# wdas03/lipreading-video-generation

Hardware: AMD Instinct MI355X
Metric: train-step frames/sec + DDIM steps/sec, 128x128x16 UNet3D at 1/2/4/8 GPUs (higher is better)
Workload: dtype bf16

## Files before the change

### include/vdiff.h

```cpp
#ifndef VDIFF_H
#define VDIFF_H

#include <stdint.h>
#include <stddef.h>

#ifdef __cplusplus
extern "C" {
#endif

#define VDIFF_ABI_VERSION 1

enum vd_status { VD_OK = 0, VD_EINVAL = 1, VD_EUNSUPPORTED = 2, VD_ELAUNCH = 3 };
enum vd_dtype { VD_F32 = 0, VD_BF16 = 1 };

int vd_version(void);
const char* vd_last_error(void);
int vd_device_info(char* buf, int buflen);

int vd_timestep_embedding(const int64_t* t, int B, int dim, float max_period,
                          float* out, void* stream);
int vd_timestep_embedding_tab(const int64_t* t, int B, int dim, const float* freqs,
                              float* out, void* stream);

int vd_q_sample(const void* x0, const void* eps, void* xt, const int64_t* t,
// ... 82 lines not shown
typedef struct vd_conv_desc {
  int B;
  int Ti, Hi, Wi, Ci;
  int To, Ho, Wo, Co;
  int kt, kh, kw;
  int st, sh, sw;
  int pt, ph, pw;
  int x_cstride;
  int y_cstride;
  int dtype;
} vd_conv_desc;

int vd_conv3d_fwd(const vd_conv_desc* d, const void* x, const void* w_fwd,
                  const float* bias, const float* chan_add,
                  const void* residual, void* y, void* stream);
int vd_conv3d_bwd_data(const vd_conv_desc* d, const void* dy,
                       const void* w_bwd, void* dx, void* stream);
int vd_conv3d_bwd_weight(const vd_conv_desc* d, const void* x, const void* dy,
                         float* dw, void* stream);
size_t vd_conv3d_bwd_weight_workspace_size(const vd_conv_desc* d);
int vd_conv3d_bwd_weight_det(const vd_conv_desc* d, const void* x, const void* dy, float* dw,
                             int Co_out, int Ci_out, void* workspace, size_t workspace_bytes,
                             void* stream);

int vd_conv_set_wgrad(int mode);
int vd_conv_set_halo(int mode);

size_t vd_channel_sums_workspace_size(int B, int C);
int vd_channel_sums(const void* x, int B, int64_t S, int C, int cstride, int dtype,
                    float* out, void* workspace, void* stream);
int vd_conv_pack_weight(const float* w, int Co, int Ci, int taps, int Cip, int Cop,
                        int transpose, int dtype, void* out, void* stream);
typedef struct {
  const float* w;
  void* out;
  int Co, Ci, taps, Cip, Cop, transpose;
  int64_t start;
} vd_pack_desc;
int vd_conv_pack_weights(const vd_pack_desc* descs, int n, int64_t total, int dtype,
                         void* stream);

typedef struct vd_attn_desc {
  int nseq, seq_len, head_dim, groups;
  int64_t batch_stride, group_stride, token_stride;
  int64_t o_batch_stride, o_group_stride, o_token_stride;
  float scale;
// ... 71 lines not shown
```

### lipreading-video-generation_amd/csrc/conv.hip

```cpp
#include "vd_common.h"
#include <stdio.h>
#include <stdlib.h>

#include <atomic>

namespace {

constexpr int kThreads = 256;
constexpr int kBK = 32;

template <typename T> struct Cfg;
template <> struct Cfg<bf16_t> {
  static constexpr int EPC = 8;
  static constexpr int CPR = kBK / EPC;
  static constexpr int LDK = kBK;
};
template <> struct Cfg<float> {
  static constexpr int EPC = 4;
  static constexpr int CPR = kBK / EPC;
  static constexpr int LDK = kBK + 4;
};

__device__ __forceinline__ int swz(int r, int kc) {
  const int t = (r >> 2) & 3;
// ... 194 lines not shown
#pragma unroll
        for (int e = 0; e < 8; ++e) o[e] += rv[e];
      }
      store8(out, o);
    } else {
      for (int e = 0; e < lim; ++e) {
        float val = o[e];
        if (residual) val += Elem<T>::ld(residual + m * g.dNs + n + e);
        Elem<T>::st(out + e, val);
      }
    }
  }
}

struct WgtGeom {
  int B;
  int Ti, Hi, Wi, Ci, xCs;
  int To, Ho, Wo, Co, yCs;
  int kt, kh, kw, st, sh, sw, pt, ph, pw;
  int64_t M;
  int64_t m_per_split;
  int64_t split_stride;
  int xcd_tiles, xcd_total;
};

__device__ __forceinline__ bool wg_tile(const WgtGeom& g, int* tile, int* split) {
  if (g.xcd_tiles == 0) {
    *tile = blockIdx.x;
    *split = blockIdx.y;
    return true;
  }
  const int per = gridDim.x / 8;
  const int L = (blockIdx.x % 8) * per + blockIdx.x / 8;
  if (L >= g.xcd_total) return false;
  *tile = L % g.xcd_tiles;
  *split = L / g.xcd_tiles;
  return true;
}

__device__ __forceinline__ void wg_out(const WgtGeom& g, float* dw, int split, int64_t off,
                                       float v) {
  if (g.split_stride)
    dw[(int64_t)split * g.split_stride + off] = v;
  else
    atomicAdd(dw + off, v);
}

template <typename T>
__global__ __launch_bounds__(kThreads) void conv_wgrad_kernel(WgtGeom g, const T* __restrict__ x,
                                                              const T* __restrict__ dy,
                                                              float* __restrict__ dw) {
  constexpr int TM = 64, TN = 64;
  constexpr int PK = 32;
  constexpr int PAD = sizeof(T) == 2 ? 8 : 4;
  constexpr int LD = TM + PAD;
  constexpr int EPC = 16 / sizeof(T);
  constexpr int CPRW = TM / EPC;
  constexpr int CH = PK * CPRW / kThreads;
  constexpr int STAGE = 2 * PK * LD;
  extern __shared__ __attribute__((aligned(16))) char smem[];
  T* lds = reinterpret_cast<T*>(smem);

  const int taps = g.kt * g.kh * g.kw;
  const int co_tiles = (g.Co + TM - 1) / TM;
  const int ci_tiles = (g.Ci + TN - 1) / TN;
  int bid = blockIdx.x;
  const int cot = bid % co_tiles; bid /= co_tiles;
  const int cit = bid % ci_tiles; bid /= ci_tiles;
  const int tap = bid;
// ... 490 lines not shown
    const int tap = tab * g.kw + tc;
#pragma unroll
    for (int i = 0; i < 2; ++i)
#pragma unroll
      for (int j = 0; j < 2; ++j) {
        const int ci = ci0 + wn * 32 + 16 * j + fr;
        if (ci >= g.Ci) continue;
#pragma unroll
        for (int r = 0; r < 4; ++r) {
          const int co = co0 + wm * 32 + 16 * i + fq * 4 + r;
          if (co < g.Co) wg_out(g, dw, blockIdx.y, (int64_t)co * krow + (int64_t)tap * g.Ci + ci, acc[tc][i][j][r]);
        }
      }
  }
}

__device__ __forceinline__ int wg_swz(int r) {
  const int u = r >> 1;
  return ((u + 2 * (u >> 2)) & 3) << 1;
}
__device__ __forceinline__ int wg_off(int r, int c) {
  return r * 64 + ((((c >> 3) ^ wg_swz(r)) << 3) | (c & 7));
}

template <int RW, int COT, int NST, bool ONE, bool PLANE = false>
__global__ __launch_bounds__(kThreads, PLANE ? 1 : 2) void wgrad_dma_kernel(
    WgtGeom g, int wc, const bf16_t* __restrict__ x, const bf16_t* __restrict__ dy,
    float* __restrict__ dw) {
  constexpr int PY = COT / 32, PX = RW / 32;
  constexpr int PIECES = PY + PX;
  constexpr int Y_BYTES = COT * 128, STAGE = (COT + RW) * 128;
  constexpr int WTM = COT / 2, NI = WTM / 16;
  constexpr int NT = ONE ? 1 : (PLANE ? 9 : 3);
  static_assert(!PLANE || RW >= 3 * 66, "plane: three strip rows of 66 pixels");
  static_assert(!ONE || RW == 64, "1x1: the X tile is the step's 64 pixels");
  extern __shared__ __attribute__((aligned(16))) char smem[];
  const bf16_t* lds = reinterpret_cast<const bf16_t*>(smem);

  const int co_tiles = (g.Co + COT - 1) / COT, ci_tiles = (g.Ci + 63) / 64;
  int bid, wsplit;
  if (!wg_tile(g, &bid, &wsplit)) return;
  const int cot = bid % co_tiles; bid /= co_tiles;
  const int cit = bid % ci_tiles; bid /= ci_tiles;
  const int tab = bid;
  const int ta = PLANE ? tab : tab / g.kh, tb = PLANE ? 0 : tab % g.kh;
  const int co0 = cot * COT, ci0 = cit * 64;
// ... 87 lines not shown
      cw += 64;
      while (cw >= g.Wo) {
        cw -= g.Wo;
        if (++chh == g.Ho) {
          chh = 0;
          if (++ct == g.To) {
            ct = 0;
            ++cb;
          }
        }
      }
    }
  };

  const int wm = wave & 1, wn = wave >> 1;
  f32x4 acc[NT][NI][2];
#pragma unroll
  for (int tc = 0; tc < NT; ++tc)
#pragma unroll
    for (int i = 0; i < NI; ++i)
#pragma unroll
      for (int j = 0; j < 2; ++j) acc[tc][i][j] = f32x4{0.f, 0.f, 0.f, 0.f};

  vm_drain();
#pragma unroll
  for (int s = 0; s < NST - 1; ++s) issue(s);
  const int fr = lane & 15, fq = lane >> 4, q4 = fr >> 2, p4 = fr & 3;
  for (int s = 0; s < nsteps; ++s) {
    vm_wait_barrier<(NST - 2) * PIECES>();
    issue(s + NST - 1);
    const bf16_t* Ys = lds + (s % NST) * (STAGE / 2);
    const bf16_t* Xs = Ys + Y_BYTES / 2;
#pragma unroll
    for (int ks = 0; ks < 2; ++ks) {
      const int p_lo = 32 * ks + 8 * fq + q4, p_hi = p_lo + 4;
      bf16x8 af[NI];
#pragma unroll
      for (int i = 0; i < NI; ++i) {
        const int c = wm * WTM + 16 * i + 4 * p4;
        const bf16_t* plane = Ys + (c >> 6) * 4096;
        const bf16x4 lo = __builtin_amdgcn_ds_read_tr16_b64_v4i16(
            (lds_bf16x4*)(plane + wg_off(p_lo, c & 63)));
        const bf16x4 hi = __builtin_amdgcn_ds_read_tr16_b64_v4i16(
            (lds_bf16x4*)(plane + wg_off(p_hi, c & 63)));
        af[i] = bf16x8{lo[0], lo[1], lo[2], lo[3], hi[0], hi[1], hi[2], hi[3]};
      }
      const int s_lo = ONE ? p_lo : (p_lo / wc) * SW + p_lo % wc;
      const int s_hi = ONE ? p_hi : (p_hi / wc) * SW + p_hi % wc;
#pragma unroll
      for (int tc = 0; tc < NT; ++tc) {
        bf16x8 bfr[2];
        const int sh_t = PLANE ? (tc / 3) * SW + tc % 3 : tc;
#pragma unroll
        for (int j = 0; j < 2; ++j) {
          const int c = wn * 32 + 16 * j + 4 * p4;
          const bf16x4 lo = __builtin_amdgcn_ds_read_tr16_b64_v4i16(
              (lds_bf16x4*)(Xs + wg_off(s_lo + sh_t, c)));
          const bf16x4 hi = __builtin_amdgcn_ds_read_tr16_b64_v4i16(
              (lds_bf16x4*)(Xs + wg_off(s_hi + sh_t, c)));
          bfr[j] = bf16x8{lo[0], lo[1], lo[2], lo[3], hi[0], hi[1], hi[2], hi[3]};
        }
#pragma unroll
        for (int i = 0; i < NI; ++i)
#pragma unroll
          for (int j = 0; j < 2; ++j)
            acc[tc][i][j] =
                __builtin_amdgcn_mfma_f32_16x16x32_bf16(af[i], bfr[j], acc[tc][i][j], 0, 0, 0);
      }
    }
  }
  vm_drain();
  const int taps = g.kt * g.kh * g.kw;
  const int64_t krow = (int64_t)taps * g.Ci;
#pragma unroll
  for (int tc = 0; tc < NT; ++tc) {
    const int tap = ONE ? 0 : (PLANE ? ta * 9 + tc : tab * g.kw + tc);
#pragma unroll
    for (int i = 0; i < NI; ++i)
#pragma unroll
      for (int j = 0; j < 2; ++j) {
        const int ci = ci0 + wn * 32 + 16 * j + fr;
        if (ci >= g.Ci) continue;
#pragma unroll
        for (int r = 0; r < 4; ++r) {
          const int co = co0 + wm * WTM + 16 * i + fq * 4 + r;
          if (co < g.Co) wg_out(g, dw, wsplit, (int64_t)co * krow + (int64_t)tap * g.Ci + ci, acc[tc][i][j][r]);
        }
      }
  }
}

template <int RW, int COT, int NST, int KIND, bool ER = true>
__global__ __launch_bounds__(kThreads, 2) void wgrad_strip_kernel(WgtGeom g, int wc,
                                                                  const bf16_t* __restrict__ x,
                                                                  const bf16_t* __restrict__ dy,
                                                                  float* __restrict__ dw) {
  constexpr int PY = COT / 32, PX = RW / 32;
  constexpr int PIECES = PY + PX;
  constexpr int Y_BYTES = COT * 128, STAGE = (COT + RW) * 128;
  constexpr bool ROW1 = KIND == 1, ONE = KIND == 2;
  constexpr int WTM = COT / 2, NI = WTM / 16, NT = ONE ? 1 : 3;
  static_assert(!ONE || RW == 64, "1x1: the X tile is the step's 64 pixels");
  extern __shared__ __attribute__((aligned(16))) char smem[];

  const int co_tiles = (g.Co + COT - 1) / COT, ci_tiles = (g.Ci + 63) / 64;
  int bid, wsplit;
  if (!wg_tile(g, &bid, &wsplit)) return;
  const int cot = bid % co_tiles; bid /= co_tiles;
  const int cit = bid % ci_tiles; bid /= ci_tiles;
  const int tab = bid;
  const int ta = tab / g.kh, tb = tab % g.kh;
  const int co0 = cot * COT, ci0 = cit * 64;
  const int64_t mbeg = (int64_t)wsplit * g.m_per_split;
  int64_t mend = mbeg + g.m_per_split;
  if (mend > g.M) mend = g.M;
  if (mbeg >= mend) return;

  const int tid = threadIdx.x, lane = tid & 63;
  const int wave = __builtin_amdgcn_readfirstlane(tid >> 6);
// ... 111 lines not shown
#pragma unroll
      for (int j = 0; j < 2; ++j) acc[tc][i][j] = f32x4{0.f, 0.f, 0.f, 0.f};
  const int fr = lane & 15, fq = lane >> 4, q4 = fr >> 2, p4 = fr & 3;
  const uint32_t lb = lds_addr(smem);
  uint32_t abase[2][2][NI], xbase[2][2][NT][2];
#pragma unroll
  for (int ks = 0; ks < 2; ++ks)
#pragma unroll
    for (int hl = 0; hl < 2; ++hl) {
      const int p = 32 * ks + 8 * fq + q4 + 4 * hl;
      const int sp = ONE ? p : (p / wc) * SW + p % wc;
#pragma unroll
      for (int i = 0; i < NI; ++i) {
        const int c = wm * WTM + 16 * i + 4 * p4;
        abase[ks][hl][i] = lb + ((c >> 6) * 4096 + wg_off(p, c & 63)) * 2;
      }
#pragma unroll
      for (int tc = 0; tc < NT; ++tc)
#pragma unroll
        for (int j = 0; j < 2; ++j)
          xbase[ks][hl][tc][j] = lb + Y_BYTES + wg_off(sp + tc, wn * 32 + 16 * j + 4 * p4) * 2;
    }

  vm_drain();
#pragma unroll
  for (int s = 0; s < NST - 1; ++s) issue(s, s);
  for (int s0 = 0; s0 < nsteps; s0 += NST) {
#pragma unroll
    for (int ks = 0; ks < 2; ++ks)
#pragma unroll
      for (int hl = 0; hl < 2; ++hl) {
#pragma unroll
        for (int i = 0; i < NI; ++i) asm volatile("" : "+v"(abase[ks][hl][i]));
#pragma unroll
        for (int tc = 0; tc < NT; ++tc)
#pragma unroll
          for (int j = 0; j < 2; ++j) asm volatile("" : "+v"(xbase[ks][hl][tc][j]));
      }
#pragma unroll
    for (int u = 0; u < NST; ++u) {
      const int s = s0 + u;
      if (s >= nsteps) break;
      vm_lgk_wait_barrier<(NST - 2) * PIECES>();
      issue(s + NST - 1, (u + NST - 1) % NST);
#pragma unroll
      for (int ks = 0; ks < 2; ++ks) {
        bf16x8 af[NI], bfr[NT][2];
        auto rd = [&](uint32_t a0, uint32_t a1) {
          const bf16x4 lo = __builtin_amdgcn_ds_read_tr16_b64_v4i16(
              (lds_bf16x4*)(uintptr_t)(a0 + u * STAGE));
          const bf16x4 hi = __builtin_amdgcn_ds_read_tr16_b64_v4i16(
              (lds_bf16x4*)(uintptr_t)(a1 + u * STAGE));
          return bf16x8{lo[0], lo[1], lo[2], lo[3], hi[0], hi[1], hi[2], hi[3]};
        };
#pragma unroll
        for (int i = 0; i < NI; ++i) af[i] = rd(abase[ks][0][i], abase[ks][1][i]);
        if constexpr (ER) {
#pragma unroll
          for (int tc = 0; tc < NT; ++tc)
#pragma unroll
            for (int j = 0; j < 2; ++j) bfr[tc][j] = rd(xbase[ks][0][tc][j], xbase[ks][1][tc][j]);
          __builtin_amdgcn_sched_barrier(0);
        }
#pragma unroll
        for (int tc = 0; tc < NT; ++tc) {
          if constexpr (!ER) {
#pragma unroll
            for (int j = 0; j < 2; ++j) bfr[tc][j] = rd(xbase[ks][0][tc][j], xbase[ks][1][tc][j]);
          }
#pragma unroll
          for (int i = 0; i < NI; ++i)
#pragma unroll
            for (int j = 0; j < 2; ++j)
              acc[tc][i][j] = __builtin_amdgcn_mfma_f32_16x16x32_bf16(af[i], bfr[tc][j],
                                                                      acc[tc][i][j], 0, 0, 0);
        }
      }
    }
  }
  vm_drain();
  const int taps = g.kt * g.kh * g.kw;
  const int64_t krow = (int64_t)taps * g.Ci;
#pragma unroll
  for (int tc = 0; tc < NT; ++tc) {
    const int tap = ONE ? 0 : tab * g.kw + tc;
#pragma unroll
    for (int i = 0; i < NI; ++i)
#pragma unroll
      for (int j = 0; j < 2; ++j) {
        const int ci = ci0 + wn * 32 + 16 * j + fr;
        if (ci >= g.Ci) continue;
#pragma unroll
        for (int r = 0; r < 4; ++r) {
          const int co = co0 + wm * WTM + 16 * i + fq * 4 + r;
          if (co < g.Co)
            wg_out(g, dw, wsplit, (int64_t)co * krow + (int64_t)tap * g.Ci + ci,
                   acc[tc][i][j][r]);
        }
      }
  }
}

template <int BM, int BN, int WAVES_M, bool TR, int NST>
__global__ __launch_bounds__(kThreads, 2) void igemm_dma_kernel(
    GemmGeom g, const bf16_t* __restrict__ src, const bf16_t* __restrict__ wt,
    bf16_t* __restrict__ dst, const float* __restrict__ bias, const float* __restrict__ chan_add,
    const bf16_t* __restrict__ residual) {
  constexpr int WAVES_N = 4 / WAVES_M;
  constexpr int WTM = BM / WAVES_M, WTN = BN / WAVES_N;
  constexpr int NI = WTM / 16, NJ = WTN / 16;
  constexpr int IA = BM / 32, IB = BN / 32;
  constexpr int PIECES = IA + IB;
  constexpr int A_BYTES = BM * 128, STAGE = (BM + BN) * 128;
  extern __shared__ __attribute__((aligned(16))) char smem[];
  const bf16_t* lds = reinterpret_cast<const bf16_t*>(smem);

  const int tid = threadIdx.x, lane = tid & 63;
  const int wave = __builtin_amdgcn_readfirstlane(tid >> 6);
  const int wm = wave % WAVES_M, wn = wave / WAVES_M;
  const int64_t m0 = (int64_t)blockIdx.x * BM;
  const int n0 = blockIdx.y * BN;
  const int C = g.sC;
  const int taps = g.kt * g.kh * g.kw, khw = g.kh * g.kw;
// ... 803 lines not shown
  int rc = check_desc(d);
  if (rc) return rc;
  VD_REQUIRE(dy && w_bwd && dx, "null tensor");
  VD_REQUIRE(d->Co % 8 == 0, "bwd_data needs Co %% 8 == 0 (got %d)", d->Co);
  VD_REQUIRE(d->y_cstride == 0 || d->y_cstride % 8 == 0, "bad y_cstride");
  GemmGeom g;
  g.B = d->B;
  g.sT = d->To; g.sH = d->Ho; g.sW = d->Wo; g.sC = d->Co;
  g.sCs = d->y_cstride ? d->y_cstride : d->Co;
  g.dT = d->Ti; g.dH = d->Hi; g.dW = d->Wi; g.N = d->Ci;
  g.dNs = d->x_cstride ? d->x_cstride : d->Ci;
  g.kt = d->kt; g.kh = d->kh; g.kw = d->kw;
  g.st = d->st; g.sh = d->sh; g.sw = d->sw;
  g.pt = d->pt; g.ph = d->ph; g.pw = d->pw;
  g.M = (int64_t)d->B * d->Ti * d->Hi * d->Wi;
  g.K = d->kt * d->kh * d->kw * d->Co;
  return VD_DISPATCH_DTYPE(d->dtype, T, {
    launch_gemm<T, true>(g, dy, w_bwd, dx, nullptr, nullptr, nullptr, VD_STREAM(stream));
  });
}

}

static int wgrad_run(const vd_conv_desc* d, const void* x, const void* dy, float* dw,
                     int64_t split_stride, int64_t* splits_out, bool dry, void* stream) {
  int rc = check_desc(d);
  if (rc) return rc;
  VD_REQUIRE(dry || (x && dy && dw), "null tensor");
  VD_REQUIRE(d->Co % 8 == 0, "bwd_weight needs Co %% 8 == 0 (got %d)", d->Co);
  WgtGeom g;
  g.split_stride = split_stride;
  g.xcd_tiles = g.xcd_total = 0;
  g.B = d->B;
  g.Ti = d->Ti; g.Hi = d->Hi; g.Wi = d->Wi; g.Ci = d->Ci;
  g.xCs = d->x_cstride ? d->x_cstride : d->Ci;
  g.To = d->To; g.Ho = d->Ho; g.Wo = d->Wo; g.Co = d->Co;
  g.yCs = d->y_cstride ? d->y_cstride : d->Co;
  g.kt = d->kt; g.kh = d->kh; g.kw = d->kw;
  g.st = d->st; g.sh = d->sh; g.sw = d->sw;
  g.pt = d->pt; g.ph = d->ph; g.pw = d->pw;
  g.M = (int64_t)d->B * d->To * d->Ho * d->Wo;
  const int taps = d->kt * d->kh * d->kw;
  const bool strip = d->dtype == VD_BF16 && !g_legacy_conv && d->kh == 3 && d->kw == 3 &&
                     (d->kt == 1 || d->kt == 3) && d->st == 1 && d->sh == 1 && d->sw == 1 &&
                     d->pt == d->kt / 2 && d->ph == 1 && d->pw == 1 &&
                     (d->Wo % 64 == 0 || (64 % d->Wo == 0 && 64 / d->Wo <= d->Ho));
  const bool one = d->dtype == VD_BF16 && !g_legacy_conv && taps == 1 && d->st == 1 &&
                   d->sh == 1 && d->sw == 1 && d->pt == 0 && d->ph == 0 && d->pw == 0;
  const int64_t x_bytes = (int64_t)d->B * d->Ti * d->Hi * d->Wi * g.xCs * 2;
  const bool dma = g_conv_dma && (strip || one) && g.xCs % 8 == 0 && g.yCs % 8 == 0 &&
                   x_bytes < (1ll << 31) && g.M * g.yCs * 2 < (1ll << 31);
  hipStream_t st = VD_STREAM(stream);
  if (dma) {
    const int wc = one ? 64 : (d->Wo < 64 ? d->Wo : 64);
    const int rows = one ? 64 : (64 / wc) * (wc + 2);
// ... 42 lines not shown
      const int64_t slots = 256 * (int64_t)std::max(1, std::min(3, 163840 / ring));
      int64_t pick = 0, fill_pick = 0;
      double best_fill = -1.0;
      for (int64_t s = std::max<int64_t>(1, splits / 3); s <= splits; ++s) {
        const int64_t sr = vd_cdiv(g.M, vd_cdiv(vd_cdiv(g.M, s), 64) * 64);
        const double r = (double)(tiles * sr) / (double)slots;
        if (r < 0.9) continue;
        const double fill = r / std::ceil(r);
        if (fill >= 0.93) { pick = s; break; }
        if (fill > best_fill + 1e-9) { best_fill = fill; fill_pick = s; }
      }
      if (!pick) pick = fill_pick;
      if (pick) splits = pick;
    }
    static const int wsplits = [] {
      const char* e = getenv("VDIFF_WGRAD_SPLITS");
      return e ? atoi(e) : 0;
    }();
    if (wsplits > 0) splits = std::min<int64_t>(wsplits, vd_cdiv(g.M, 64));
    if (splits < 1) splits = 1;
    g.m_per_split = vd_cdiv(vd_cdiv(g.M, splits), 64) * 64;
    splits = vd_cdiv(g.M, g.m_per_split);
    *splits_out = splits;
    if (dry) return VD_OK;
    dim3 grid((unsigned)tiles, (unsigned)splits);
    static const int wxcd = [] {
      const char* e = getenv("VDIFF_WGRAD_XCD");
      return e ? atoi(e) : 1;
    }();
    if (wxcd && tiles > 1) {
      g.xcd_tiles = (int)tiles;
      g.xcd_total = (int)(tiles * splits);
      grid = dim3((unsigned)vd_cdiv(tiles * splits, 8) * 8, 1);
    }
#define VD_WGD(RW, COT, NST, ONE, ...)                                                     \
  do {                                                                                     \
    auto kern = wgrad_dma_kernel<RW, COT, NST, ONE, ##__VA_ARGS__>;                        \
    const int lds = NST * (COT + RW) * 128;                                                \
    (void)hipFuncSetAttribute((const void*)kern,                                           \
                              hipFuncAttributeMaxDynamicSharedMemorySize, lds);            \
    kern<<<grid, kThreads, lds, st>>>(g, wc, (const bf16_t*)x, (const bf16_t*)dy, dw);     \
  } while (0)
#define VD_WG1(COT, NST)                                                                   \
  do {                                                                                     \
     \
    auto kern = wgrad_strip_kernel<64, COT, NST, 2, false>;                                \
// ... 83 lines not shown
    if (rows <= 96) VD_WG(96);
    else if (rows <= 128) VD_WG(128);
    else VD_WG(192);
#undef VD_WG
    return vd::check_launch("conv_wgrad");
  }
  const int64_t tiles = (int64_t)vd_cdiv(d->Co, 64) * vd_cdiv(d->Ci, 64) * taps;
  int64_t splits = vd_cdiv(2048, tiles);
  int64_t maxs = vd_cdiv(g.M, 512);
  if (splits > maxs) splits = maxs;
  if (splits < 1) splits = 1;
  g.m_per_split = vd_cdiv(vd_cdiv(g.M, splits), 32) * 32;
  splits = vd_cdiv(g.M, g.m_per_split);
  *splits_out = splits;
  if (dry) return VD_OK;
  return VD_DISPATCH_DTYPE(d->dtype, T, {
    constexpr int LD = 64 + (sizeof(T) == 2 ? 8 : 4);
    const size_t lds = 2 * 2 * 32 * LD * sizeof(T);
    conv_wgrad_kernel<T><<<dim3((unsigned)tiles, (unsigned)splits), kThreads, lds,
                           VD_STREAM(stream)>>>(g, (const T*)x, (const T*)dy, dw);
  });
}

__global__ __launch_bounds__(256) void wgrad_finish_kernel(const float* __restrict__ part,
                                                           int splits, int64_t sstride, int Ci,
                                                           int taps, int Co_out, int Ci_out,
                                                           float* __restrict__ out) {
  __shared__ float4 sums[16][17];
  const int oi = threadIdx.x & 15, grp = threadIdx.x >> 4;
  const int64_t i = (int64_t)blockIdx.x * 16 + oi;
  const int ci4 = Ci / 4;
  const int64_t n4 = (int64_t)Co_out * taps * ci4;
  const int64_t row = i / ci4;
  const int ci = (int)(i % ci4) * 4;
  float4 a = make_float4(0.f, 0.f, 0.f, 0.f);
  auto add = [&](const float4& v) {
    a.x += v.x;
    a.y += v.y;
    a.z += v.z;
    a.w += v.w;
  };
  if (i < n4 && ci < Ci_out) {
    const float* p = part + row * Ci + ci;
    int sp = grp;
    for (; sp + 48 < splits; sp += 64) {
      float4 v[4];
#pragma unroll
      for (int u = 0; u < 4; ++u)
        v[u] = *reinterpret_cast<const float4*>(p + (int64_t)(sp + 16 * u) * sstride);
#pragma unroll
      for (int u = 0; u < 4; ++u) add(v[u]);
    }
    for (; sp < splits; sp += 16) add(*reinterpret_cast<const float4*>(p + (int64_t)sp * sstride));
  }
  sums[grp][oi] = a;
  __syncthreads();
  if (grp != 0 || i >= n4 || ci >= Ci_out) return;
  a = sums[0][oi];
  for (int k = 1; k < 16; ++k) {
    const float4 v = sums[k][oi];
    a.x += v.x;
    a.y += v.y;
    a.z += v.z;
    a.w += v.w;
  }
  const int tap = (int)(row % taps), co = (int)(row / taps);
  float* o = out + ((int64_t)co * Ci_out + ci) * taps + tap;
  const float av[4] = {a.x, a.y, a.z, a.w};
#pragma unroll
  for (int k = 0; k < 4; ++k)
    if (ci + k < Ci_out) o[(int64_t)k * taps] = av[k];
}

extern "C" {

int vd_conv3d_bwd_weight(const vd_conv_desc* d, const void* x, const void* dy, float* dw,
                         void* stream) {
  int64_t splits = 0;
  return wgrad_run(d, x, dy, dw, 0, &splits, false, stream);
}

size_t vd_conv3d_bwd_weight_workspace_size(const vd_conv_desc* d) {
  int64_t splits = 0;
  if (!d || wgrad_run(d, nullptr, nullptr, nullptr, 1, &splits, true, nullptr)) return 0;
  return (size_t)splits * d->Co * d->kt * d->kh * d->kw * d->Ci * sizeof(float) + 256;
}

int vd_conv3d_bwd_weight_det(const vd_conv_desc* d, const void* x, const void* dy, float* dw,
                             int Co_out, int Ci_out, void* workspace, size_t workspace_bytes,
                             void* stream) {
  int64_t splits = 0;
  int rc = wgrad_run(d, x, dy, nullptr, 1, &splits, true, stream);
  if (rc) return rc;
  VD_REQUIRE(x && dy && dw && workspace, "null tensor");
  VD_REQUIRE(Co_out > 0 && Co_out <= d->Co && Ci_out > 0 && Ci_out <= d->Ci,
             "dw extent %dx%d outside the descriptor's %dx%d", Co_out, Ci_out, d->Co, d->Ci);
  VD_REQUIRE(d->Ci % 4 == 0, "bwd_weight_det needs Ci %% 4 == 0 (got %d)", d->Ci);
  VD_REQUIRE((reinterpret_cast<uintptr_t>(workspace) & 15) == 0, "workspace not 16-B aligned");
  const int taps = d->kt * d->kh * d->kw;
  const int64_t sstride = (int64_t)d->Co * taps * d->Ci;
  VD_REQUIRE(workspace_bytes >= (size_t)splits * sstride * sizeof(float),
             "workspace %zu B < %lld B", workspace_bytes,
             (long long)(splits * sstride * (int64_t)sizeof(float)));
  float* part = reinterpret_cast<float*>(workspace);
  rc = wgrad_run(d, x, dy, part, sstride, &splits, false, stream);
  if (rc) return rc;
  const int64_t n4 = (int64_t)Co_out * taps * (d->Ci / 4);
  wgrad_finish_kernel<<<(unsigned)vd_cdiv(n4, 16), 256, 0, VD_STREAM(stream)>>>(
      part, (int)splits, sstride, d->Ci, taps, Co_out, Ci_out, dw);
  return vd::check_launch("conv_wgrad_finish");
}

}
```

### lipreading-video-generation_amd/vdiff/_lib.py

```python
from __future__ import annotations

import ctypes as C
import os
import threading

_HERE = os.path.dirname(os.path.abspath(__file__))
LIB_PATH = os.environ.get("VDIFF_LIB") or os.path.join(_HERE, "libvdiff.so")

VD_F32 = 0
VD_BF16 = 1
ABI_VERSION = 1

_vp = C.c_void_p
_i = C.c_int
_i64 = C.c_int64
_u64 = C.c_uint64
_f = C.c_float
_sz = C.c_size_t


class ConvDesc(C.Structure):
    _fields_ = [(n, _i) for n in (
        "B", "Ti", "Hi", "Wi", "Ci", "To", "Ho", "Wo", "Co",
        "kt", "kh", "kw", "st", "sh", "sw", "pt", "ph", "pw",
# ... 37 lines not shown
    "vd_groupnorm_silu_bwd": (_i, [_vp, _vp, _vp, _vp, _vp, _vp, _vp, _vp, _vp, _i, _i64, _i, _i,
                                   _i, _f, _u64, _i, _vp, _vp]),
    "vd_groupnorm_silu_bwd_add": (_i, [_vp, _vp, _vp, _vp, _vp, _vp, _vp, _vp, _vp, _vp, _i, _i64,
                                       _i, _i, _i, _f, _u64, _i, _vp, _vp]),
    "vd_silu": (_i, [_vp, _vp, _i64, _i, _vp]),
    "vd_silu_bwd": (_i, [_vp, _vp, _vp, _i64, _i, _vp]),
    "vd_cond_concat": (_i, [_vp, _vp, _vp, _vp, _i, _i, _i, _i, _i, _i, _i, _i, _i, _i, _i, _vp]),
    "vd_cond_concat_bwd_workspace_size": (_sz, [_i, _i, _i, _i, _i]),
    "vd_cond_concat_bwd": (_i, [_vp, _vp, _vp, _i, _i, _i, _i, _i, _i, _i, _i, _i, _i, _i, _vp,
                                _vp]),
    "vd_upsample_nearest_hw": (_i, [_vp, _vp, _i, _i, _i, _i, _i, _i, _vp]),
    "vd_upsample_nearest_hw_bwd": (_i, [_vp, _vp, _i, _i, _i, _i, _i, _i, _vp]),
    "vd_channel_sums_workspace_size": (_sz, [_i, _i]),
    "vd_channel_sums": (_i, [_vp, _i, _i64, _i, _i, _i, _vp, _vp, _vp]),
    "vd_conv_pack_weight": (_i, [_vp, _i, _i, _i, _i, _i, _i, _i, _vp, _vp]),
    "vd_conv_pack_weights": (_i, [_vp, _i, _i64, _i, _vp]),
    "vd_conv_set_wgrad": (_i, [C.c_int]),
    "vd_conv_set_halo": (_i, [_i]),
    "vd_conv3d_fwd": (_i, [C.POINTER(ConvDesc), _vp, _vp, _vp, _vp, _vp, _vp, _vp]),
    "vd_conv3d_bwd_data": (_i, [C.POINTER(ConvDesc), _vp, _vp, _vp, _vp]),
    "vd_conv3d_bwd_weight": (_i, [C.POINTER(ConvDesc), _vp, _vp, _vp, _vp]),
    "vd_conv3d_bwd_weight_workspace_size": (_sz, [C.POINTER(ConvDesc)]),
    "vd_conv3d_bwd_weight_det": (_i, [C.POINTER(ConvDesc), _vp, _vp, _vp, _i, _i, _vp, _sz, _vp]),
    "vd_attention_fwd": (_i, [C.POINTER(AttnDesc), _vp, _vp, _vp, _vp, _vp, _vp]),
    "vd_attention_fwd_workspace_size": (_sz, [C.POINTER(AttnDesc)]),
    "vd_attention_fwd_ws": (_i, [C.POINTER(AttnDesc), _vp, _vp, _vp, _vp, _vp, _vp, _sz, _vp]),
    "vd_attention_bwd_workspace_size": (_sz, [C.POINTER(AttnDesc)]),
    "vd_attention_set_config": (C.c_int, [C.c_int]),
    "vd_attention_bwd": (_i, [C.POINTER(AttnDesc), _vp, _vp, _vp, _vp, _vp, _vp, _vp, _vp, _vp,
                              _vp, _vp]),
    "vd_attention_bwd_dq": (_i, [C.POINTER(AttnDesc), _vp, _vp, _vp, _vp, _vp, _vp, _vp, _vp,
                                 _vp]),
    "vd_attention_bwd_dkdv": (_i, [C.POINTER(AttnDesc), _vp, _vp, _vp, _vp, _vp, _vp, _vp, _vp,
                                   _vp]),
    "vd_cross_attention_fwd_workspace_size": (_sz, [C.POINTER(XAttnDesc)]),
    "vd_cross_attention_fwd": (_i, [C.POINTER(XAttnDesc), _vp, _vp, _vp, _vp, _vp, _vp, _sz,
                                    _vp]),
    "vd_cross_attention_bwd_workspace_size": (_sz, [C.POINTER(XAttnDesc)]),
    "vd_cross_attention_bwd_dq": (_i, [C.POINTER(XAttnDesc), _vp, _vp, _vp, _vp, _vp, _vp, _vp,
                                       _vp, _vp]),
    "vd_cross_attention_bwd_dkdv": (_i, [C.POINTER(XAttnDesc), _vp, _vp, _vp, _vp, _vp, _vp,
                                         _vp, _vp, _vp]),
    "vd_resize_plan": (_i, [_i, _i, _vp, _vp, _i]),
    "vd_frames_resize_normalize": (_i, [_vp, _i64, _i, _i, _i, _i, _vp, _vp, _i, _vp, _vp, _i,
                                        _vp, _vp, _i, _i64, _i, _vp]),
    "vd_audio_window": (_i, [_vp, _i, _i64, _i, C.c_double, _i, _i, _i, _i, _i, _vp]),
# ... 53 lines not shown
```

### lipreading-video-generation_amd/vdiff/ops.py

```python
from __future__ import annotations

import math
import os
from typing import Optional, Sequence, Tuple

import torch

from . import _lib
from ._lib import AttnDesc, ConvDesc, VD_BF16, VD_F32, XAttnDesc

_DT = {torch.float32: VD_F32, torch.bfloat16: VD_BF16}
_WGRAD_ATOMIC = os.environ.get("VDIFF_WGRAD_ATOMIC", "0") == "1"


def _p(t: Optional[torch.Tensor]):
    return None if t is None else t.data_ptr()


def _stream(t: torch.Tensor):
    return torch.cuda.current_stream(t.device).cuda_stream


def _dtype(t: torch.Tensor) -> int:
    try:
        return _DT[t.dtype]
    except KeyError:
        raise TypeError(f"libvdiff supports float32/bfloat16 activations, got {t.dtype}") from None


def _gpu(*ts):
    for t in ts:
        if t is not None and not t.is_cuda:
            raise RuntimeError("libvdiff ops run on the GPU only (got a CPU tensor; there is no "
                               "CPU fallback in the product path)")

# ... 619 lines not shown
        out = torch.empty(B, cp, dtype=torch.float32, device=x.device)
        ws = torch.empty(_lib.lib().vd_channel_sums_workspace_size(B, cp), dtype=torch.uint8,
                         device=x.device)
        _lib.call("vd_channel_sums", _p(x), B, S, cp, 0, _dtype(x), _p(out), _p(ws), _stream(x))
        return out[:, :Cc]
    parts = []
    for c0 in range(0, cp, 2048):
        w = min(2048, cp - c0)
        o = torch.empty(B, w, dtype=torch.float32, device=x.device)
        ws = torch.empty(_lib.lib().vd_channel_sums_workspace_size(B, w), dtype=torch.uint8,
                         device=x.device)
        _lib.call("vd_channel_sums", x.data_ptr() + c0 * x.element_size(), B, S, w, cp,
                  _dtype(x), _p(o), _p(ws), _stream(x))
        parts.append(o)
    return torch.cat(parts, dim=1)[:, :Cc]


def _conv_key(Ci, Co, k, s, out):
    return f"{Ci}->{Co} k{'x'.join(map(str, k))} s{'x'.join(map(str, s))} out{'x'.join(map(str, out))}"


def _conv_flop(B, out, Co, k, Ci):
    return 2.0 * B * out[0] * out[1] * out[2] * Co * k[0] * k[1] * k[2] * Ci


class ConvFn(torch.autograd.Function):

    @staticmethod
    def forward(ctx, x, weight, bias, chan_add, residual, stride, padding):
        _gpu(x, weight)
        x = to_cl(x)
        dt = x.dtype
        Co, Ci = weight.shape[:2]
        if x.shape[1] != Ci:
            raise ValueError(f"conv expects {Ci} input channels, got {x.shape[1]}")
        nd, k, s, p, sp, out = _geom(x.shape, weight.shape, stride, padding)
        B = x.shape[0]
        taps = k[0] * k[1] * k[2]
        Cip = (Ci + 7) // 8 * 8
        xp = _pad_channels(x, Cip)
        w_fwd = _pack_weight(weight, Co, Ci, taps, Cip, Co, False, dt)
        ys = [B, Co] + out[3 - nd:] if nd > 0 else [B, Co]
        y = empty_cl(ys, dt, x.device)
        b32 = None if bias is None else bias.detach().float().contiguous()
        ca = None if chan_add is None else chan_add.detach().float().reshape(B, Co).contiguous()
        res = None
# ... 26 lines not shown
        d = _desc(B, sp, Cip, out, Co, k, s, p, _DT[dt])
        dx = dw = db = dca = dres = None
        st = _stream(dy)
        Cop = (Co + 7) // 8 * 8
        dyp = _pad_channels(dy, Cop)
        if Cop != Co:
            d = _desc(B, sp, Cip, out, Cop, k, s, p, _DT[dt])
        if ctx.needs_input_grad[0]:
            w_bwd = _pack_weight(weight, Co, Ci, taps, Cip, Cop, True, dt)
            dxp = empty_cl([B, Cip] + xshape[2:], dt, dy.device)
            ev = _timer.begin() if _timer is not None and _timer.convs else None
            if dt == torch.bfloat16 and any(v > 1 for v in s):
                uo = [sp[i] + 2 * p[i] - k[i] + 1 for i in range(3)]
                dyd = zeros_cl([B, Cop] + uo, dt, dy.device)
                dyd[:, :, ::s[0], ::s[1], ::s[2]] = dyp.reshape([B, Cop] + list(out))
                d1 = _desc(B, sp, Cip, uo, Cop, k, [1, 1, 1], p, _DT[dt])
                _lib.call("vd_conv3d_bwd_data", d1, _p(dyd), _p(w_bwd), _p(dxp), st)
            else:
                _lib.call("vd_conv3d_bwd_data", d, _p(dyp), _p(w_bwd), _p(dxp), st)
            if ev is not None:
                _timer.end_conv(ev, "conv_bwd_data", _conv_key(Cip, Co, k, s, out),
                                _conv_flop(B, out, Co, k, Ci))
            dx = dxp[:, :Ci] if Cip != Ci else dxp
        if ctx.needs_input_grad[1]:
            ev = _timer.begin() if _timer is not None and _timer.convs else None
            if _WGRAD_ATOMIC:
                dwp = torch.zeros(Cop, taps, Cip, dtype=torch.float32, device=dy.device)
                _lib.call("vd_conv3d_bwd_weight", d, _p(xp), _p(dyp), _p(dwp), st)
                dw = dwp[:Co, :, :Ci].permute(0, 2, 1).reshape(weight.shape)
            else:
                dw = torch.empty(weight.shape, dtype=torch.float32, device=dy.device)
                ws = torch.empty(_lib.lib().vd_conv3d_bwd_weight_workspace_size(d),
                                 dtype=torch.uint8, device=dy.device)
                _lib.call("vd_conv3d_bwd_weight_det", d, _p(xp), _p(dyp), _p(dw), Co, Ci,
                          _p(ws), ws.numel(), st)
            if ev is not None:
                _timer.end_conv(ev, "conv_bwd_weight", _conv_key(Cip, Co, k, s, out),
                                _conv_flop(B, out, Co, k, Ci))
            dw = dw.to(weight.dtype)
        want_b = has_b and ctx.needs_input_grad[2]
        want_ca = has_ca and ctx.needs_input_grad[3]
        if want_b or want_ca:
            sums = channel_sums(dyp)[:, :Co]
            if want_b:
                db = (sums[0] if B == 1 else sums.sum(0)).to(bdt)
            if want_ca:
                dca = sums.reshape(ca_shape)
        if has_res and ctx.needs_input_grad[4]:
            dres = dy
        return dx, dw, db, dca, dres, None, None


def conv(x, weight, bias=None, stride=1, padding=0, chan_add=None, residual=None):
    nd = weight.dim() - 2
    if isinstance(stride, int):
        stride = (stride,) * nd
    if isinstance(padding, int):
        padding = (padding,) * nd
    return ConvFn.apply(x, weight, bias, chan_add, residual, tuple(stride), tuple(padding))


class KernelTimer:

    def __init__(self, attention=True, convs=True):
        self.attention, self.convs = attention, convs
        self.records = []
# ... 247 lines not shown
```

Before: 46.37.

## Fold bias/channel-add gradient sums into the weight-gradient kernels

Computes the per-batch channel sums of dy (needed for bias and chan_add gradients) inside the 1x1 DMA and strip weight-gradient kernels, reading the dy tiles already staged in LDS. Partial sums per split, batch slot and wave go to the workspace and are reduced by extra blocks in the existing finish kernel. This removes the separate channel_sums pass over dy. In exchange it adds register pressure and per-step accumulation work to the wgrad inner loop, and needs a larger workspace. Shapes the fold does not cover still fall back to channel_sums.

```diff
diff --git a/include/vdiff.h b/include/vdiff.h
--- a/include/vdiff.h
+++ b/include/vdiff.h
@@ -128,6 +128,11 @@
 int vd_conv3d_bwd_weight_det(const vd_conv_desc* d, const void* x, const void* dy, float* dw,
                              int Co_out, int Ci_out, void* workspace, size_t workspace_bytes,
                              void* stream);
+size_t vd_conv3d_bwd_weight_bias_workspace_size(const vd_conv_desc* d);
+int vd_conv3d_bwd_weight_bias_det(const vd_conv_desc* d, const void* x, const void* dy,
+                                  float* dw, int Co_out, int Ci_out, float* dsum,
+                                  void* workspace, size_t workspace_bytes, void* stream);
+int vd_conv_set_bias_fold(int mode);
 
 int vd_conv_set_wgrad(int mode);
 int vd_conv_set_halo(int mode);
diff --git a/lipreading-video-generation_amd/csrc/conv.hip b/lipreading-video-generation_amd/csrc/conv.hip
--- a/lipreading-video-generation_amd/csrc/conv.hip
+++ b/lipreading-video-generation_amd/csrc/conv.hip
@@ -240,6 +240,8 @@
   int64_t m_per_split;
   int64_t split_stride;
   int xcd_tiles, xcd_total;
+  float* bsum;
+  int bs_k, bs_ns;
 };
 
 __device__ __forceinline__ bool wg_tile(const WgtGeom& g, int* tile, int* split) {
@@ -263,6 +265,87 @@
   else
     atomicAdd(dw + off, v);
 }
+
+__device__ __forceinline__ void bf_add(float (&a)[8], const uint4& r) {
+  const uint32_t w[4] = {r.x, r.y, r.z, r.w};
+#pragma unroll
+  for (int e = 0; e < 4; ++e) {
+    a[2 * e] += __uint_as_float(w[e] << 16);
+    a[2 * e + 1] += __uint_as_float(w[e] & 0xffff0000u);
+  }
+}
+
+template <int NPT, int NR, int RS>
+struct BiasFold {
+  int bbeg, bend;
+  int k;
+  float a[NPT][8];
+
+  __device__ __forceinline__ void init(const WgtGeom& g, int mbeg) {
+    const int thw = g.To * g.Ho * g.Wo;
+    bbeg = mbeg / thw * thw;
+    bend = bbeg + thw;
+    k = 0;
+    clear();
+  }
+  __device__ __forceinline__ void clear() {
+#pragma unroll
+    for (int q = 0; q < NPT; ++q)
+#pragma unroll
+      for (int e = 0; e < 8; ++e) a[q][e] = 0.f;
+  }
+  __device__ __forceinline__ void flush(const WgtGeom& g, int split, int sigma, int lane,
+                                        int cbase) {
+#pragma unroll
+    for (int q = 0; q < NPT; ++q)
+#pragma unroll
+      for (int e = 0; e < 8; ++e) {
+        float v = a[q][e];
+        v += __shfl_xor(v, 8);
+        v += __shfl_xor(v, 16);
+        v += __shfl_xor(v, 32);
+        a[q][e] = v;
+      }
+    if (lane < 8) {
+      float* o = g.bsum + (((int64_t)split * g.bs_k + k) * g.bs_ns + sigma) * g.Co;
+#pragma unroll
+      for (int q = 0; q < NPT; ++q) {
+        const int c = cbase + q * 64 + lane * 8;
+        if (c < g.Co) {
+          *reinterpret_cast<float4*>(o + c) = make_float4(a[q][0], a[q][1], a[q][2], a[q][3]);
+          *reinterpret_cast<float4*>(o + c + 4) = make_float4(a[q][4], a[q][5], a[q][6], a[q][7]);
+        }
+      }
+    }
+    clear();
+  }
+  template <typename Ld>
+  __device__ __forceinline__ void step(const WgtGeom& g, int ms, int me, int row0, int split,
+                                       int sigma, int lane, int cbase, Ld ld) {
+    if (ms >= bbeg && ms + 64 <= bend) {
+#pragma unroll
+      for (int i = 0; i < NR; ++i)
+#pragma unroll
+        for (int q = 0; q < NPT; ++q) bf_add(a[q], ld(q, i));
+      return;
+    }
+    for (;;) {
+#pragma unroll
+      for (int i = 0; i < NR; ++i) {
+        const int p = ms + row0 + RS * i;
+        if (p >= bbeg && p < bend) {
+#pragma unroll
+          for (int q = 0; q < NPT; ++q) bf_add(a[q], ld(q, i));
+        }
+      }
+      if (ms + 64 <= bend || bend >= me) return;
+      flush(g, split, sigma, lane, cbase);
+      bbeg = bend;
+      bend += g.To * g.Ho * g.Wo;
+      ++k;
+    }
+  }
+};
 
 template <typename T>
 __global__ __launch_bounds__(kThreads) void conv_wgrad_kernel(WgtGeom g, const T* __restrict__ x,
@@ -799,6 +882,20 @@
 __device__ __forceinline__ int wg_off(int r, int c) {
   return r * 64 + ((((c >> 3) ^ wg_swz(r)) << 3) | (c & 7));
 }
+
+template <int COT>
+struct BfTile {
+  static constexpr int NP = COT / 64;
+  static constexpr bool SPLIT = NP == 2;
+  static constexpr int NPT = SPLIT ? 1 : NP, RS = SPLIT ? 16 : 32, NR = 64 / RS;
+  static constexpr int NS = SPLIT ? 2 : 4;
+  using Fold = BiasFold<NPT, NR, RS>;
+  __device__ static __forceinline__ int row0(int tid) {
+    return SPLIT ? ((tid >> 7) * 8 + ((tid & 63) >> 3)) : (tid >> 3);
+  }
+  __device__ static __forceinline__ int plane0(int tid) { return SPLIT ? ((tid >> 6) & 1) : 0; }
+  __device__ static __forceinline__ int sigma(int wave) { return SPLIT ? (wave >> 1) : wave; }
+};
 
 template <int RW, int COT, int NST, bool ONE, bool PLANE = false>
 __global__ __launch_bounds__(kThreads, PLANE ? 1 : 2) void wgrad_dma_kernel(
@@ -932,6 +1029,13 @@
 #pragma unroll
       for (int j = 0; j < 2; ++j) acc[tc][i][j] = f32x4{0.f, 0.f, 0.f, 0.f};
 
+  using BT = BfTile<COT>;
+  const bool fold = ONE && g.bsum != nullptr && cit == 0;
+  typename BT::Fold bf;
+  if constexpr (ONE) bf.init(g, (int)mbeg);
+  const int bf_row0 = BT::row0(tid), bf_cb = co0 + BT::plane0(tid) * 64;
+  const int bf_off = BT::plane0(tid) * 4096 + wg_off(bf_row0, (lane & 7) * 8);
+
   vm_drain();
 #pragma unroll
   for (int s = 0; s < NST - 1; ++s) issue(s);
@@ -941,6 +1045,13 @@
     issue(s + NST - 1);
     const bf16_t* Ys = lds + (s % NST) * (STAGE / 2);
     const bf16_t* Xs = Ys + Y_BYTES / 2;
+    if constexpr (ONE)
+      if (fold)
+        bf.step(g, (int)mbeg + s * 64, (int)mend, bf_row0, wsplit, BT::sigma(wave), lane, bf_cb,
+                [&](int q, int i) {
+                  return *reinterpret_cast<const uint4*>(Ys + bf_off + q * 4096 +
+                                                         i * BT::RS * 64);
+                });
 #pragma unroll
     for (int ks = 0; ks < 2; ++ks) {
       const int p_lo = 32 * ks + 8 * fq + q4, p_hi = p_lo + 4;
@@ -980,6 +1091,8 @@
     }
   }
   vm_drain();
+  if constexpr (ONE)
+    if (fold) bf.flush(g, wsplit, BT::sigma(wave), lane, bf_cb);
   const int taps = g.kt * g.kh * g.kw;
   const int64_t krow = (int64_t)taps * g.Ci;
 #pragma unroll
@@ -1000,11 +1113,11 @@
   }
 }
 
-template <int RW, int COT, int NST, int KIND, bool ER = true>
-__global__ __launch_bounds__(kThreads, 2) void wgrad_strip_kernel(WgtGeom g, int wc,
-                                                                  const bf16_t* __restrict__ x,
-                                                                  const bf16_t* __restrict__ dy,
-                                                                  float* __restrict__ dw) {
+template <int RW, int COT, int NST, int KIND, bool ER, bool FOLD>
+__device__ __forceinline__ void wgrad_strip_body(const WgtGeom& g, int wc,
+                                                 const bf16_t* __restrict__ x,
+                                                 const bf16_t* __restrict__ dy,
+                                                 float* __restrict__ dw) {
   constexpr int PY = COT / 32, PX = RW / 32;
   constexpr int PIECES = PY + PX;
   constexpr int Y_BYTES = COT * 128, STAGE = (COT + RW) * 128;
@@ -1162,6 +1275,12 @@
           xbase[ks][hl][tc][j] = lb + Y_BYTES + wg_off(sp + tc, wn * 32 + 16 * j + 4 * p4) * 2;
     }
 
+  using BT = BfTile<COT>;
+  typename BT::Fold bf;
+  if constexpr (FOLD) bf.init(g, ms0);
+  const int bf_row0 = BT::row0(tid), bf_cb = co0 + BT::plane0(tid) * 64;
+  const char* bf_src = smem + (BT::plane0(tid) * 4096 + wg_off(bf_row0, (lane & 7) * 8)) * 2;
+
   vm_drain();
 #pragma unroll
   for (int s = 0; s < NST - 1; ++s) issue(s, s);
@@ -1183,6 +1302,12 @@
       if (s >= nsteps) break;
       vm_lgk_wait_barrier<(NST - 2) * PIECES>();
       issue(s + NST - 1, (u + NST - 1) % NST);
+      if constexpr (FOLD)
+        bf.step(g, ms0 + s * 64, me, bf_row0, wsplit, BT::sigma(wave), lane, bf_cb,
+                [&](int q, int i) {
+                  return *reinterpret_cast<const uint4*>(bf_src + u * STAGE + q * 8192 +
+                                                         i * BT::RS * 128);
+                });
 #pragma unroll
       for (int ks = 0; ks < 2; ++ks) {
         bf16x8 af[NI], bfr[NT][2];
@@ -1219,6 +1344,7 @@
     }
   }
   vm_drain();
+  if constexpr (FOLD) bf.flush(g, wsplit, BT::sigma(wave), lane, bf_cb);
   const int taps = g.kt * g.kh * g.kw;
   const int64_t krow = (int64_t)taps * g.Ci;
 #pragma unroll
@@ -1239,6 +1365,21 @@
         }
       }
   }
+}
+
+template <int RW, int COT, int NST, int KIND, bool ER = true>
+__global__ __launch_bounds__(kThreads, 2) void wgrad_strip_kernel(WgtGeom g, int wc,
+                                                                  const bf16_t* __restrict__ x,
+                                                                  const bf16_t* __restrict__ dy,
+                                                                  float* __restrict__ dw) {
+  if constexpr (KIND == 2) {
+    int bid, wsplit;
+    if (g.bsum != nullptr && wg_tile(g, &bid, &wsplit) && bid < (g.Co + COT - 1) / COT) {
+      wgrad_strip_body<RW, COT, NST, KIND, ER, true>(g, wc, x, dy, dw);
+      return;
+    }
+  }
+  wgrad_strip_body<RW, COT, NST, KIND, ER, false>(g, wc, x, dy, dw);
 }
 
 template <int BM, int BN, int WAVES_M, bool TR, int NST>
@@ -2088,8 +2229,13 @@
 
 }
 
+struct BiasSlots {
+  int k, ns;
+  int64_t m_per_split;
+};
 static int wgrad_run(const vd_conv_desc* d, const void* x, const void* dy, float* dw,
-                     int64_t split_stride, int64_t* splits_out, bool dry, void* stream) {
+                     int64_t split_stride, int64_t* splits_out, bool dry, void* stream,
+                     float* bsum = nullptr, BiasSlots* bs_out = nullptr) {
   int rc = check_desc(d);
   if (rc) return rc;
   VD_REQUIRE(dry || (x && dy && dw), "null tensor");
@@ -2097,6 +2243,9 @@
   WgtGeom g;
   g.split_stride = split_stride;
   g.xcd_tiles = g.xcd_total = 0;
+  g.bsum = nullptr;
+  g.bs_k = g.bs_ns = 0;
+  if (bs_out) *bs_out = BiasSlots{0, 0, 0};
   g.B = d->B;
   g.Ti = d->Ti; g.Hi = d->Hi; g.Wi = d->Wi; g.Ci = d->Ci;
   g.xCs = d->x_cstride ? d->x_cstride : d->Ci;
@@ -2185,6 +2334,13 @@
     g.m_per_split = vd_cdiv(vd_cdiv(g.M, splits), 64) * 64;
     splits = vd_cdiv(g.M, g.m_per_split);
     *splits_out = splits;
+    if (one) {
+      const int64_t thw = (int64_t)d->To * d->Ho * d->Wo;
+      g.bsum = bsum;
+      g.bs_k = (int)std::min<int64_t>(d->B, (g.m_per_split - 1) / thw + 2);
+      g.bs_ns = cot == 128 ? 2 : 4;
+      if (bs_out) *bs_out = BiasSlots{g.bs_k, g.bs_ns, g.m_per_split};
+    }
     if (dry) return VD_OK;
     dim3 grid((unsigned)tiles, (unsigned)splits);
     static const int wxcd = [] {
@@ -2314,12 +2470,60 @@
   });
 }
 
+struct BiasFinish {
+  unsigned dw_blocks;
+  const float* bsum;
+  float* dsum;
+  int B, Co, bs_k, ns;
+  int64_t thw, m_per_split;
+};
+
 __global__ __launch_bounds__(256) void wgrad_finish_kernel(const float* __restrict__ part,
                                                            int splits, int64_t sstride, int Ci,
                                                            int taps, int Co_out, int Ci_out,
-                                                           float* __restrict__ out) {
+                                                           float* __restrict__ out,
+                                                           BiasFinish bf) {
   __shared__ float4 sums[16][17];
   const int oi = threadIdx.x & 15, grp = threadIdx.x >> 4;
+  if (blockIdx.x >= bf.dw_blocks) {
+    float4* flat = &sums[0][0];
+    const int o4 = threadIdx.x & 3, g64 = threadIdx.x >> 2;
+    const int64_t i = (int64_t)(blockIdx.x - bf.dw_blocks) * 4 + o4;
+    const int c4 = bf.Co / 4;
+    const bool live = i < (int64_t)bf.B * c4;
+    float4 a = make_float4(0.f, 0.f, 0.f, 0.f);
+    auto add = [&](const float4& v) {
+      a.x += v.x;
+      a.y += v.y;
+      a.z += v.z;
+      a.w += v.w;
+    };
+    if (live) {
+      const int b = (int)(i / c4), c = (int)(i % c4) * 4;
+      const int64_t s0 = b * bf.thw / bf.m_per_split;
+      const int64_t s1 = ((b + 1) * bf.thw - 1) / bf.m_per_split;
+      for (int64_t sp = s0 + g64; sp <= s1; sp += 64) {
+        const int k = b - (int)(sp * bf.m_per_split / bf.thw);
+        const float* p = bf.bsum + ((sp * bf.bs_k + k) * bf.ns) * bf.Co + c;
+        for (int w = 0; w < bf.ns; ++w)
+          add(*reinterpret_cast<const float4*>(p + (int64_t)w * bf.Co));
+      }
+    }
+    flat[g64 * 4 + o4] = a;
+    __syncthreads();
+    if (g64 < 8) {
+      a = flat[g64 * 32 + o4];
+      for (int k = 1; k < 8; ++k) add(flat[(g64 * 8 + k) * 4 + o4]);
+    }
+    __syncthreads();
+    if (g64 < 8) flat[g64 * 4 + o4] = a;
+    __syncthreads();
+    if (g64 != 0 || !live) return;
+    a = flat[o4];
+    for (int k = 1; k < 8; ++k) add(flat[k * 4 + o4]);
+    *reinterpret_cast<float4*>(bf.dsum + i * 4) = a;
+    return;
+  }
   const int64_t i = (int64_t)blockIdx.x * 16 + oi;
   const int ci4 = Ci / 4;
   const int64_t n4 = (int64_t)Co_out * taps * ci4;
@@ -2364,6 +2568,12 @@
     if (ci + k < Ci_out) o[(int64_t)k * taps] = av[k];
 }
 
+static std::atomic<int> g_bias_fold{1};
+
+static int wgrad_det(const vd_conv_desc* d, const void* x, const void* dy, float* dw, int Co_out,
+                     int Ci_out, float* dsum, void* workspace, size_t workspace_bytes,
+                     void* stream);
+
 extern "C" {
 
 int vd_conv3d_bwd_weight(const vd_conv_desc* d, const void* x, const void* dy, float* dw,
@@ -2378,11 +2588,48 @@
   return (size_t)splits * d->Co * d->kt * d->kh * d->kw * d->Ci * sizeof(float) + 256;
 }
 
+int vd_conv_set_bias_fold(int mode) {
+  if (mode == -1) return g_bias_fold.load(std::memory_order_relaxed);
+  if (mode != 0 && mode != 1) {
+    (void)vd::fail(VD_EINVAL, "conv bias fold mode %d (0, 1; -1 reads it)", mode);
+    return -2;
+  }
+  return g_bias_fold.exchange(mode);
+}
+
+size_t vd_conv3d_bwd_weight_bias_workspace_size(const vd_conv_desc* d) {
+  int64_t splits = 0;
+  BiasSlots bs{0, 0, 0};
+  if (!d || wgrad_run(d, nullptr, nullptr, nullptr, 1, &splits, true, nullptr, nullptr, &bs))
+    return 0;
+  const size_t extra = bs.k ? (size_t)splits * bs.k * bs.ns * d->Co * sizeof(float)
+                            : vd_channel_sums_workspace_size(d->B, d->Co);
+  return (size_t)splits * d->Co * d->kt * d->kh * d->kw * d->Ci * sizeof(float) + extra + 256;
+}
+
 int vd_conv3d_bwd_weight_det(const vd_conv_desc* d, const void* x, const void* dy, float* dw,
                              int Co_out, int Ci_out, void* workspace, size_t workspace_bytes,
                              void* stream) {
+  return wgrad_det(d, x, dy, dw, Co_out, Ci_out, nullptr, workspace, workspace_bytes, stream);
+}
+
+int vd_conv3d_bwd_weight_bias_det(const vd_conv_desc* d, const void* x, const void* dy, float* dw,
+                                  int Co_out, int Ci_out, float* dsum, void* workspace,
+                                  size_t workspace_bytes, void* stream) {
+  VD_REQUIRE(!dsum || g_bias_fold.load(std::memory_order_relaxed),
+             "bias fold is switched off (vd_conv_set_bias_fold)");
+  VD_REQUIRE((reinterpret_cast<uintptr_t>(dsum) & 15) == 0, "dsum not 16-B aligned");
+  return wgrad_det(d, x, dy, dw, Co_out, Ci_out, dsum, workspace, workspace_bytes, stream);
+}
+
+}
+
+static int wgrad_det(const vd_conv_desc* d, const void* x, const void* dy, float* dw, int Co_out,
+                     int Ci_out, float* dsum, void* workspace, size_t workspace_bytes,
+                     void* stream) {
   int64_t splits = 0;
-  int rc = wgrad_run(d, x, dy, nullptr, 1, &splits, true, stream);
+  BiasSlots bs{0, 0, 0};
+  int rc = wgrad_run(d, x, dy, nullptr, 1, &splits, true, stream, nullptr, &bs);
   if (rc) return rc;
   VD_REQUIRE(x && dy && dw && workspace, "null tensor");
   VD_REQUIRE(Co_out > 0 && Co_out <= d->Co && Ci_out > 0 && Ci_out <= d->Ci,
@@ -2391,16 +2638,36 @@
   VD_REQUIRE((reinterpret_cast<uintptr_t>(workspace) & 15) == 0, "workspace not 16-B aligned");
   const int taps = d->kt * d->kh * d->kw;
   const int64_t sstride = (int64_t)d->Co * taps * d->Ci;
-  VD_REQUIRE(workspace_bytes >= (size_t)splits * sstride * sizeof(float),
-             "workspace %zu B < %lld B", workspace_bytes,
-             (long long)(splits * sstride * (int64_t)sizeof(float)));
+  const int64_t part_n = splits * sstride;
+  const bool folds = dsum && bs.k > 0;
+  const size_t extra = !dsum ? 0
+                       : folds ? (size_t)splits * bs.k * bs.ns * d->Co * sizeof(float)
+                               : vd_channel_sums_workspace_size(d->B, d->Co);
+  VD_REQUIRE(workspace_bytes >= (size_t)part_n * sizeof(float) + extra,
+             "workspace %zu B < %zu B", workspace_bytes, (size_t)part_n * sizeof(float) + extra);
   float* part = reinterpret_cast<float*>(workspace);
-  rc = wgrad_run(d, x, dy, part, sstride, &splits, false, stream);
+  float* bsum = folds ? part + part_n : nullptr;
+  rc = wgrad_run(d, x, dy, part, sstride, &splits, false, stream, bsum);
   if (rc) return rc;
   const int64_t n4 = (int64_t)Co_out * taps * (d->Ci / 4);
-  wgrad_finish_kernel<<<(unsigned)vd_cdiv(n4, 16), 256, 0, VD_STREAM(stream)>>>(
-      part, (int)splits, sstride, d->Ci, taps, Co_out, Ci_out, dw);
-  return vd::check_launch("conv_wgrad_finish");
-}
-
-}
+  BiasFinish bf{};
+  bf.dw_blocks = (unsigned)vd_cdiv(n4, 16);
+  unsigned blocks = bf.dw_blocks;
+  if (folds) {
+    bf.bsum = bsum;
+    bf.dsum = dsum;
+    bf.B = d->B;
+    bf.Co = d->Co;
+    bf.bs_k = bs.k;
+    bf.ns = bs.ns;
+    bf.thw = (int64_t)d->To * d->Ho * d->Wo;
+    bf.m_per_split = bs.m_per_split;
+    blocks += (unsigned)vd_cdiv((int64_t)d->B * (d->Co / 4), 4);
+  }
+  wgrad_finish_kernel<<<blocks, 256, 0, VD_STREAM(stream)>>>(
+      part, (int)splits, sstride, d->Ci, taps, Co_out, Ci_out, dw, bf);
+  rc = vd::check_launch("conv_wgrad_finish");
+  if (rc || !dsum || folds) return rc;
+  return vd_channel_sums(dy, d->B, (int64_t)d->To * d->Ho * d->Wo, d->Co, d->y_cstride, d->dtype,
+                         dsum, part + part_n, stream);
+}
diff --git a/lipreading-video-generation_amd/vdiff/_lib.py b/lipreading-video-generation_amd/vdiff/_lib.py
--- a/lipreading-video-generation_amd/vdiff/_lib.py
+++ b/lipreading-video-generation_amd/vdiff/_lib.py
@@ -83,6 +83,10 @@
     "vd_conv3d_bwd_weight": (_i, [C.POINTER(ConvDesc), _vp, _vp, _vp, _vp]),
     "vd_conv3d_bwd_weight_workspace_size": (_sz, [C.POINTER(ConvDesc)]),
     "vd_conv3d_bwd_weight_det": (_i, [C.POINTER(ConvDesc), _vp, _vp, _vp, _i, _i, _vp, _sz, _vp]),
+    "vd_conv3d_bwd_weight_bias_workspace_size": (_sz, [C.POINTER(ConvDesc)]),
+    "vd_conv3d_bwd_weight_bias_det": (_i, [C.POINTER(ConvDesc), _vp, _vp, _vp, _i, _i, _vp, _vp,
+                                           _sz, _vp]),
+    "vd_conv_set_bias_fold": (_i, [C.c_int]),
     "vd_attention_fwd": (_i, [C.POINTER(AttnDesc), _vp, _vp, _vp, _vp, _vp, _vp]),
     "vd_attention_fwd_workspace_size": (_sz, [C.POINTER(AttnDesc)]),
     "vd_attention_fwd_ws": (_i, [C.POINTER(AttnDesc), _vp, _vp, _vp, _vp, _vp, _vp, _sz, _vp]),
diff --git a/lipreading-video-generation_amd/vdiff/ops.py b/lipreading-video-generation_amd/vdiff/ops.py
--- a/lipreading-video-generation_amd/vdiff/ops.py
+++ b/lipreading-video-generation_amd/vdiff/ops.py
@@ -11,6 +11,14 @@
 
 _DT = {torch.float32: VD_F32, torch.bfloat16: VD_BF16}
 _WGRAD_ATOMIC = os.environ.get("VDIFF_WGRAD_ATOMIC", "0") == "1"
+
+
+def bias_fold() -> bool:
+    return _lib.lib().vd_conv_set_bias_fold(-1) == 1
+
+
+def set_bias_fold(on: bool) -> bool:
+    return _lib.lib().vd_conv_set_bias_fold(1 if on else 0) == 1
 
 
 def _p(t: Optional[torch.Tensor]):
@@ -676,6 +684,16 @@
 
 def _conv_flop(B, out, Co, k, Ci):
     return 2.0 * B * out[0] * out[1] * out[2] * Co * k[0] * k[1] * k[2] * Ci
+
+
+def conv_wgrad_bias(d, xp, dyp, wshape):
+    dw = torch.empty(wshape, dtype=torch.float32, device=dyp.device)
+    sums = torch.empty(d.B, d.Co, dtype=torch.float32, device=dyp.device)
+    ws = torch.empty(_lib.lib().vd_conv3d_bwd_weight_bias_workspace_size(d), dtype=torch.uint8,
+                     device=dyp.device)
+    _lib.call("vd_conv3d_bwd_weight_bias_det", d, _p(xp), _p(dyp), _p(dw), wshape[0], wshape[1],
+              _p(sums), _p(ws), ws.numel(), _stream(dyp))
+    return dw, sums
 
 
 class ConvFn(torch.autograd.Function):
@@ -748,12 +766,18 @@
                 _timer.end_conv(ev, "conv_bwd_data", _conv_key(Cip, Co, k, s, out),
                                 _conv_flop(B, out, Co, k, Ci))
             dx = dxp[:, :Ci] if Cip != Ci else dxp
+        want_b = has_b and ctx.needs_input_grad[2]
+        want_ca = has_ca and ctx.needs_input_grad[3]
+        sums = None
         if ctx.needs_input_grad[1]:
             ev = _timer.begin() if _timer is not None and _timer.convs else None
             if _WGRAD_ATOMIC:
                 dwp = torch.zeros(Cop, taps, Cip, dtype=torch.float32, device=dy.device)
                 _lib.call("vd_conv3d_bwd_weight", d, _p(xp), _p(dyp), _p(dwp), st)
                 dw = dwp[:Co, :, :Ci].permute(0, 2, 1).reshape(weight.shape)
+            elif (want_b or want_ca) and Cop <= 2048 and bias_fold():
+                dw, sums = conv_wgrad_bias(d, xp, dyp, weight.shape)
+                sums = sums[:, :Co]
             else:
                 dw = torch.empty(weight.shape, dtype=torch.float32, device=dy.device)
                 ws = torch.empty(_lib.lib().vd_conv3d_bwd_weight_workspace_size(d),
@@ -764,10 +788,9 @@
                 _timer.end_conv(ev, "conv_bwd_weight", _conv_key(Cip, Co, k, s, out),
                                 _conv_flop(B, out, Co, k, Ci))
             dw = dw.to(weight.dtype)
-        want_b = has_b and ctx.needs_input_grad[2]
-        want_ca = has_ca and ctx.needs_input_grad[3]
         if want_b or want_ca:
-            sums = channel_sums(dyp)[:, :Co]
+            if sums is None:
+                sums = channel_sums(dyp)[:, :Co]
             if want_b:
                 db = (sums[0] if B == 1 else sums.sum(0)).to(bdt)
             if want_ca:
```

Measured after the change: 46.42 (median of 6 runs). About the same (+0.1%).
